# zjkang/Relation-DETR

Hardware: AMD Instinct MI355X
Metric: images/sec @ 800×1333, 300 queries, R50 4-level; achieved HBM GB/s (higher is better)
Workload: dtype bf16; 1 GPU; relation_detr_resnet50_800_1333 transformer stack from feature pyramids: 6 encoder layers (MSDA self-attn, S=22323, 4 levels) + two-stage top-k + 6 decoder layers (relation-biased self-attn + MSDA cross-attn + box refinement) + top-300 detections; backbone/neck excluded; batch_per_gpu=4, global_batch=4, queries=900, levels=4, launch=hipGraph replay, streams=2, gemm_tuning=False, parallelism=image-parallel x1

## Files before the change

include/relation_detr_amd.h:

```cpp
#ifndef RELATION_DETR_AMD_H
#define RELATION_DETR_AMD_H

#include <stdint.h>

#ifdef __cplusplus
extern "C" {
#endif

#define RDETR_ABI_VERSION 3

typedef enum rdetr_status {
    RDETR_OK = 0,
    RDETR_ERR_INVALID_ARG = -1,
    RDETR_ERR_UNSUPPORTED = -2,
    RDETR_ERR_LAUNCH = -3
} rdetr_status;

int rdetr_abi_version(void);
const char *rdetr_status_string(int status);

int rdetr_msda_forward_f32(const float *value, const int64_t *spatial_shapes, const int64_t *level_start_index,
                           const float *sampling_loc, const float *attn_weight, int B, int S, int H, int D,
                           int L, int Nq, int P, float *out, void *stream);

// ... 58 lines not shown
                                   int D, uint16_t *dst, void *stream);

int rdetr_linear_k256_hm_bf16(const uint16_t *x, long long ldx, const uint16_t *w, const uint16_t *bias, const uint8_t *row_mask,
                              int B, int S, uint16_t *out_hm, void *stream);

int rdetr_msda_fast_path(int H, int D, int L, int P);

int rdetr_msda_backward_f32(const float *value, const int64_t *spatial_shapes, const int64_t *level_start_index,
                            const float *sampling_loc, const float *attn_weight, const float *grad_out, int B,
                            int S, int H, int D, int L, int Nq, int P, float *grad_value,
                            float *grad_sampling_loc, float *grad_attn_weight, void *stream);

long long rdetr_msda_backward_det_workspace_bytes(int B, int S, int H, int D, int L, int Nq, int P);
int rdetr_msda_backward_det_f32(const float *value, const int64_t *spatial_shapes, const int64_t *level_start_index,
                                const float *sampling_loc, const float *attn_weight, const float *grad_out, int B, int S, int H, int D,
                                int L, int Nq, int P, void *workspace, long long workspace_bytes, float *grad_value,
                                float *grad_sampling_loc, float *grad_attn_weight, void *stream);

int rdetr_msda_backward_fused_f32(const float *value, const int64_t *spatial_shapes, const int64_t *level_start_index,
                                  const float *sampling_offsets, const float *attn_logits, const float *reference_points, int ref_dim,
                                  const float *grad_out, int B, int S, int H, int D, int L, int Nq, int P, void *workspace,
                                  long long workspace_bytes, float *grad_value, float *grad_offsets, float *grad_logits,
                                  float *grad_ref_partial, void *stream);
int rdetr_msda_backward_fused_bf16(const uint16_t *value, const int64_t *spatial_shapes, const int64_t *level_start_index,
                                   const uint16_t *sampling_offsets, const uint16_t *attn_logits, const float *reference_points,
                                   int ref_dim, const uint16_t *grad_out, int B, int S, int H, int D, int L, int Nq, int P,
                                   void *workspace, long long workspace_bytes, float *grad_value, uint16_t *grad_offsets,
                                   uint16_t *grad_logits, float *grad_ref_partial, void *stream);

int rdetr_relation_bias_f32(const float *src, const float *tgt, const float *proj_weight, const float *proj_bias,
                            int B, int N1, int N2, int Hh, int F, float scale, float temperature, float eps,
                            float *out, void *stream);

int rdetr_relation_bias_ws_f32(const float *src, const float *tgt, const float *proj_weight, const float *proj_bias,
                               int B, int N1, int N2, int Hh, int F, float scale, float temperature, float eps,
                               float *workspace, float *out, void *stream);

long long rdetr_relation_bias_backward_workspace_bytes(int B, int N1, int N2);
int rdetr_relation_bias_backward_f32(const float *src, const float *tgt, const float *grad_out, const uint8_t *active, int B, int N1,
                                     int N2, int Hh, int F, float scale, float temperature, float eps, float *workspace,
                                     float *grad_weight, float *grad_bias, void *stream);

int rdetr_bias_softmax_f32(float *scores, const float *bias, const uint8_t *mask, int BH, int N1, int N2,
                           void *stream);

int rdetr_relation_attention_bf16(const uint16_t *q, const uint16_t *k, const uint16_t *v, int ldq, int ldk, int ldv,
                                  const float *bias, const uint8_t *bool_mask, int B, int H, int D, int N, int M,
                                  float scale, uint16_t *out, int ldo, void *stream);

int rdetr_relation_attention_train_bf16(const uint16_t *q, const uint16_t *k, const uint16_t *v, int ldq, int ldk, int ldv,
                                        const float *bias, const uint8_t *bool_mask, int B, int H, int D, int N, int M,
                                        float scale, uint16_t *out, int ldo, float *lse, void *stream);

long long rdetr_relation_attention_backward_workspace_bytes(int B, int H, int N);
int rdetr_relation_attention_backward_bf16(const uint16_t *q, const uint16_t *k, const uint16_t *v, int ldq, int ldk, int ldv,
                                           const uint16_t *out, int ldo, const float *lse, const uint16_t *dout, int lddo,
                                           const float *bias, const uint8_t *bool_mask, int B, int H, int D, int N, int M,
                                           float scale, void *workspace, long long workspace_bytes, uint16_t *dq, int lddq,
                                           uint16_t *dk, int lddk, uint16_t *dv, int lddv, float *dbias, void *stream);

int rdetr_relation_attention_boxes_bf16(const uint16_t *q, const uint16_t *k, const uint16_t *v, int ldq, int ldk, int ldv,
                                        const float *src_boxes, const float *tgt_boxes, const float *proj_weight,
                                        const float *proj_bias, const uint8_t *bool_mask, int B, int H, int D,
                                        int N, int M, int F, float rel_scale, float temperature, float eps, float attn_scale,
                                        uint16_t *out, int ldo, void *stream);

int rdetr_relation_attention_boxes_train_bf16(const uint16_t *q, const uint16_t *k, const uint16_t *v, int ldq, int ldk, int ldv,
                                              const float *src_boxes, const float *tgt_boxes, const float *proj_weight,
                                              const float *proj_bias, const uint8_t *bool_mask, int B, int H, int D,
                                              int N, int M, int F, float rel_scale, float temperature, float eps, float attn_scale,
                                              uint16_t *out, int ldo, float *lse, void *stream);

long long rdetr_relation_attention_boxes_backward_workspace_bytes(int B, int H, int N, int M);
int rdetr_relation_attention_boxes_backward_bf16(const uint16_t *q, const uint16_t *k, const uint16_t *v, int ldq, int ldk, int ldv,
                                                 const uint16_t *out, int ldo, const float *lse, const uint16_t *dout, int lddo,
                                                 const float *src_boxes, const float *tgt_boxes, const float *proj_weight,
                                                 const float *proj_bias, const uint8_t *bool_mask, int B, int H, int D, int N, int M,
                                                 int F, float rel_scale, float temperature, float eps, float attn_scale,
                                                 void *workspace, long long workspace_bytes, uint16_t *dq, int lddq, uint16_t *dk,
                                                 int lddk, uint16_t *dv, int lddv, float *grad_weight, float *grad_bias,
                                                 void *stream);

int rdetr_add_layernorm_f32(const float *x, const float *residual, const float *gamma, const float *beta,
                            long long rows, int C, float eps, float *out, void *stream);
int rdetr_add_layernorm_bf16(const uint16_t *x, const uint16_t *residual, const uint16_t *gamma, const uint16_t *beta,
                             long long rows, int C, float eps, uint16_t *out, void *stream);
int rdetr_add_layernorm_strided_f32(const float *x, const float *residual, const float *gamma, const float *beta,
                                    long long rows, int C, long long ldx, long long ldr, long long ldo, float eps,
                                    float *out, void *stream);
int rdetr_add_layernorm_strided_bf16(const uint16_t *x, const uint16_t *residual, const uint16_t *gamma,
                                     const uint16_t *beta, long long rows, int C, long long ldx, long long ldr,
                                     long long ldo, float eps, uint16_t *out, void *stream);

int rdetr_add_layernorm_pos_f32(const float *x, const float *residual, const float *gamma, const float *beta,
                                const float *pos, long long rows, int C, long long ldx, long long ldr, long long ldo,
                                long long ldp, long long ldo2, float eps, float *out, float *out2, void *stream);
int rdetr_add_layernorm_pos_bf16(const uint16_t *x, const uint16_t *residual, const uint16_t *gamma,
                                 const uint16_t *beta, const uint16_t *pos, long long rows, int C, long long ldx,
                                 long long ldr, long long ldo, long long ldp, long long ldo2, float eps, uint16_t *out,
                                 uint16_t *out2, void *stream);

int rdetr_box_refine_f32(const void *delta, int delta_is_bf16, const float *ref, long long n, float eps, float *out,
                         void *stream);
int rdetr_sine_pos_embed(const float *pos, long long rows, int n, int F, float temperature, float scale, void *out,
                         int out_is_bf16, void *stream);

int rdetr_zero_masked_rows(void *x, const unsigned char *mask, long long rows, int row_bytes, long long ld_bytes,
                           void *stream);
int rdetr_row_max(const void *x, int is_bf16, long long rows, int C, long long ldx, void *out, void *stream);

long long rdetr_topk_workspace_bytes(int rows, int n, int k);
int rdetr_topk(const void *x, int is_bf16, int rows, int n, int k, void *workspace, float *values, long long *indices, void *stream);

int rdetr_box_head_k256_bf16(const uint16_t *xa, long long lda, const uint16_t *xb, long long ldb, const uint16_t *pw1,
                             const uint16_t *b1, const uint16_t *pw2, const uint16_t *b2, const uint16_t *w3, const uint16_t *b3,
                             const float *reference, int reference_is_logit, float eps, long long M, float *out_a, float *out_b,
                             void *stream);

int rdetr_query_pos_k256_bf16(const uint16_t *emb, long long lde, const uint16_t *query, long long ldq, const uint16_t *pw1a,
                              const uint16_t *pw1b, const uint16_t *b1, const uint16_t *pw2, const uint16_t *b2, const uint16_t *pv1,
                              const uint16_t *c1, const uint16_t *pv2, const uint16_t *c2, long long M, uint16_t *out_pos,
                              uint16_t *out_qpp, void *stream);

int rdetr_encoder_proj_k256_bf16(const uint16_t *x, long long ldx, const uint16_t *xq, long long ldq, const uint16_t *pwv,
                                 const uint16_t *bv, const uint16_t *pwq, const uint16_t *bq, const uint8_t *row_mask, int B, int S,
                                 int q_cols, uint16_t *out_hm, uint16_t *out_q, void *stream);

int rdetr_detections_from_topk(const float *score, const long long *index, const float *boxes, const long long *image_sizes, int B,
                               int N, int C, int K, float *out, void *stream);

int rdetr_scaled_pos(const void *a, const void *scale, const void *query, long long n, int is_bf16, void *pos, void *qp, void *stream);

int rdetr_decoder_reference(const float *reference, const float *valid_ratios, int B, int N, int L, int F, float temperature,
                            float scale, float *ref_in, void *emb, int emb_is_bf16, void *stream);

int rdetr_pyramid_points(const unsigned char *const *level_masks, const int *level_hw, int L, int B, const unsigned char *pad_mask,
                         int keep_is_bf16, float *valid_ratios, float *reference, float *logit, void *keep, void *stream);
int rdetr_nchw_to_tokens(const void *src, const void *add_vec, int is_bf16, int B, int C, int P,
                         long long out_image_stride, long long ld_out, void *out, void *stream);
int rdetr_nchw_levels_to_tokens(const void *const *level_src, const void *const *level_vec, const int *level_pixels, int L,
                                int is_bf16, int B, int C, long long out_image_stride, long long ld_out, void *out, void *stream);

int rdetr_linear_k256_bf16(const uint16_t *x, long long ldx, const uint16_t *w, const uint16_t *bias, long long M, int N,
                           int relu, uint16_t *out, long long ldo, void *stream);

int rdetr_linear_pack_k256_bf16(const uint16_t *w, uint16_t *packed, void *stream);
int rdetr_linear_ln_k256_bf16(const uint16_t *x, long long ldx, const uint16_t *packed, const uint16_t *bias,
                              const uint16_t *residual, long long ldr, const uint16_t *gamma, const uint16_t *beta, float eps,
                              long long M, uint16_t *out, long long ldo, void *stream);

int rdetr_ffn_k256_pack_bf16(const uint16_t *w1, const uint16_t *w2, int F, uint16_t *packed, void *stream);
int rdetr_ffn_k256_bf16(const uint16_t *x, long long ldx, const uint16_t *packed, const uint16_t *b1, const uint16_t *b2,
                        long long M, int F, uint16_t *out, long long ldo, void *stream);
int rdetr_ffn_ln_k256_bf16(const uint16_t *x, long long ldx, const uint16_t *packed, const uint16_t *b1, const uint16_t *b2,
                           const uint16_t *gamma, const uint16_t *beta, float eps, const uint16_t *pos, long long ldp,
                           long long M, int F, uint16_t *out, long long ldo, uint16_t *out2, long long ldo2, void *stream);
int rdetr_ffn_k256_train_bf16(const uint16_t *x, long long ldx, const uint16_t *packed, const uint16_t *b1, const uint16_t *b2,
                              long long M, int F, uint16_t *out, long long ldo, uint16_t *hid, long long ldh, void *stream);
int rdetr_ffn_k256_backward_bf16(const uint16_t *dy, long long lddy, const uint16_t *packed_t, const uint16_t *hid, long long ldh,
                                 long long M, int F, uint16_t *dh, long long ldd, uint16_t *dx, long long lddx, void *stream);

#ifdef __cplusplus
}
#endif
#endif
```

relation_detr_amd/_lib.py:

```python
from __future__ import annotations

import ctypes
import os

_HERE = os.path.dirname(os.path.abspath(__file__))
LIB_PATH = os.environ.get("RDETR_LIB_PATH") or os.path.join(_HERE, "librelation_detr_amd.so")

_c_int, _c_float, _vp, _c_ll = ctypes.c_int, ctypes.c_float, ctypes.c_void_p, ctypes.c_longlong

SIGNATURES = {
    "rdetr_abi_version": [],
    "rdetr_status_string": [_c_int],
    "rdetr_msda_fast_path": [_c_int] * 4,
    "rdetr_msda_levels_window_ok": [_vp, _vp, _c_int, _c_ll],
    "rdetr_msda_forward_f32": [_vp] * 5 + [_c_int] * 7 + [_vp, _vp],
    "rdetr_msda_forward_bf16": [_vp] * 5 + [_c_int] * 7 + [_vp, _vp],
    "rdetr_msda_forward_fused_f32": [_vp] * 6 + [_c_int] * 8 + [_vp, _vp],
    "rdetr_msda_forward_fused_bf16": [_vp] * 6 + [_c_int] * 8 + [_vp, _vp],
    "rdetr_msda_forward_fused_ex_f32": [_vp] * 4 + [_c_int, _vp, _c_int, _vp, _c_int, _vp] + [_c_int] * 7 + [_vp, _vp],
    "rdetr_msda_forward_fused_ex_bf16": [_vp] * 4 + [_c_int, _vp, _c_int, _vp, _c_int, _vp] + [_c_int] * 7 + [_vp, _vp],
    "rdetr_msda_forward_opt_bf16": [_vp, _c_int] + [_vp] * 4 + [_c_int] * 8 + [_vp, _vp],
    "rdetr_msda_forward_sweep_bf16": [_vp, _c_int] + [_vp] * 4 + [_c_int] * 7 + [_vp, _vp],
    "rdetr_msda_forward_resident_bf16": [_vp] * 5 + [_c_int] * 7 + [_vp, _vp],
    "rdetr_msda_forward_fused_resident_bf16": [_vp, _vp, _vp, _vp, _c_int, _vp, _c_int, _vp, _c_int] + [_c_int] * 7 + [_vp, _vp],
    "rdetr_msda_forward_fused_opt_bf16": [_vp, _c_int, _vp, _vp, _vp, _c_int, _vp, _c_int, _vp, _c_int, _vp] + [_c_int] * 8 + [_vp, _vp],
    "rdetr_msda_forward_fused_strided_bf16": [_vp, _c_ll, _vp, _vp, _vp, _c_int, _vp, _c_int, _vp, _c_int, _vp] + [_c_int] * 7 + [_vp, _vp],
    "rdetr_value_to_head_major_bf16": [_vp, _c_ll, _vp] + [_c_int] * 4 + [_vp, _vp],
    "rdetr_msda_backward_f32": [_vp] * 6 + [_c_int] * 7 + [_vp] * 4,
    "rdetr_msda_backward_det_workspace_bytes": [_c_int] * 7,
    "rdetr_msda_backward_det_f32": [_vp] * 6 + [_c_int] * 7 + [_vp, _c_ll] + [_vp] * 4,
    "rdetr_msda_backward_fused_f32": [_vp] * 6 + [_c_int, _vp] + [_c_int] * 7 + [_vp, _c_ll] + [_vp] * 5,
    "rdetr_msda_backward_fused_bf16": [_vp] * 6 + [_c_int, _vp] + [_c_int] * 7 + [_vp, _c_ll] + [_vp] * 5,
    "rdetr_relation_bias_f32": [_vp] * 4 + [_c_int] * 5 + [_c_float] * 3 + [_vp, _vp],
    "rdetr_relation_bias_ws_f32": [_vp] * 4 + [_c_int] * 5 + [_c_float] * 3 + [_vp, _vp, _vp],
    "rdetr_relation_bias_backward_workspace_bytes": [_c_int] * 3,
    "rdetr_relation_bias_backward_f32": [_vp] * 4 + [_c_int] * 5 + [_c_float] * 3 + [_vp] * 4,
    "rdetr_bias_softmax_f32": [_vp] * 3 + [_c_int] * 3 + [_vp],
    "rdetr_relation_attention_bf16": [_vp] * 3 + [_c_int] * 3 + [_vp, _vp] + [_c_int] * 5 + [_c_float, _vp, _c_int, _vp],
    "rdetr_relation_attention_train_bf16": [_vp] * 3 + [_c_int] * 3 + [_vp, _vp] + [_c_int] * 5 + [_c_float, _vp, _c_int, _vp, _vp],
    "rdetr_relation_attention_backward_workspace_bytes": [_c_int] * 3,
    "rdetr_relation_attention_backward_bf16": [_vp] * 3 + [_c_int] * 3 + [_vp, _c_int, _vp, _vp, _c_int, _vp, _vp] + [_c_int] * 5
                                              + [_c_float, _vp, _c_ll] + [_vp, _c_int] * 3 + [_vp, _vp],
    "rdetr_relation_attention_boxes_bf16": [_vp] * 3 + [_c_int] * 3 + [_vp] * 5 + [_c_int] * 6 + [_c_float] * 4 + [_vp, _c_int, _vp],
    "rdetr_relation_attention_boxes_train_bf16": [_vp] * 3 + [_c_int] * 3 + [_vp] * 5 + [_c_int] * 6 + [_c_float] * 4
                                                 + [_vp, _c_int, _vp, _vp],
    "rdetr_relation_attention_boxes_backward_workspace_bytes": [_c_int] * 4,
    "rdetr_relation_attention_boxes_backward_bf16": [_vp] * 3 + [_c_int] * 3 + [_vp, _c_int, _vp, _vp, _c_int] + [_vp] * 5 + [_c_int] * 6
                                                    + [_c_float] * 4 + [_vp, _c_ll] + [_vp, _c_int] * 3 + [_vp, _vp, _vp],
    "rdetr_box_refine_f32": [_vp, _c_int, _vp, _c_ll, _c_float, _vp, _vp],
    "rdetr_sine_pos_embed": [_vp, _c_ll, _c_int, _c_int, _c_float, _c_float, _vp, _c_int, _vp],
    "rdetr_zero_masked_rows": [_vp, _vp, _c_ll, _c_int, _c_ll, _vp],
    "rdetr_row_max": [_vp, _c_int, _c_ll, _c_int, _c_ll, _vp, _vp],
    "rdetr_topk_workspace_bytes": [_c_int, _c_int, _c_int],
    "rdetr_topk": [_vp, _c_int, _c_int, _c_int, _c_int, _vp, _vp, _vp, _vp],
    "rdetr_box_head_k256_bf16": [_vp, _c_ll, _vp, _c_ll, _vp, _vp, _vp, _vp, _vp, _vp, _vp, _c_int, _c_float, _c_ll, _vp, _vp, _vp],
    "rdetr_query_pos_k256_bf16": [_vp, _c_ll, _vp, _c_ll] + [_vp] * 9 + [_c_ll, _vp, _vp, _vp],
    "rdetr_encoder_proj_k256_bf16": [_vp, _c_ll, _vp, _c_ll] + [_vp] * 5 + [_c_int, _c_int, _c_int, _vp, _vp, _vp],
    "rdetr_detections_from_topk": [_vp, _vp, _vp, _vp, _c_int, _c_int, _c_int, _c_int, _vp, _vp],
    "rdetr_scaled_pos": [_vp, _vp, _vp, _c_ll, _c_int, _vp, _vp, _vp],
    "rdetr_decoder_reference": [_vp, _vp, _c_int, _c_int, _c_int, _c_int, _c_float, _c_float, _vp, _vp, _c_int, _vp],
    "rdetr_pyramid_points": [_vp, _vp, _c_int, _c_int, _vp, _c_int, _vp, _vp, _vp, _vp, _vp],
    "rdetr_linear_k256_bf16": [_vp, _c_ll, _vp, _vp, _c_ll, _c_int, _c_int, _vp, _c_ll, _vp],
    "rdetr_linear_k256_hm_bf16": [_vp, _c_ll, _vp, _vp, _vp, _c_int, _c_int, _vp, _vp],
    "rdetr_linear_pack_k256_bf16": [_vp, _vp, _vp],
    "rdetr_linear_ln_k256_bf16": [_vp, _c_ll, _vp, _vp, _vp, _c_ll, _vp, _vp, _c_float, _c_ll, _vp, _c_ll, _vp],
    "rdetr_ffn_k256_pack_bf16": [_vp, _vp, _c_int, _vp, _vp],
    "rdetr_ffn_k256_bf16": [_vp, _c_ll, _vp, _vp, _vp, _c_ll, _c_int, _vp, _c_ll, _vp],
    "rdetr_ffn_ln_k256_bf16": [_vp, _c_ll, _vp, _vp, _vp, _vp, _vp, _c_float, _vp, _c_ll, _c_ll, _c_int, _vp, _c_ll, _vp, _c_ll, _vp],
    "rdetr_ffn_k256_train_bf16": [_vp, _c_ll, _vp, _vp, _vp, _c_ll, _c_int, _vp, _c_ll, _vp, _c_ll, _vp],
    "rdetr_ffn_k256_backward_bf16": [_vp, _c_ll, _vp, _vp, _c_ll, _c_ll, _c_int, _vp, _c_ll, _vp, _c_ll, _vp],
    "rdetr_nchw_to_tokens": [_vp, _vp, _c_int, _c_int, _c_int, _c_int, _c_ll, _c_ll, _vp, _vp],
    "rdetr_nchw_levels_to_tokens": [_vp, _vp, _vp, _c_int, _c_int, _c_int, _c_int, _c_ll, _c_ll, _vp, _vp],
    "rdetr_add_layernorm_f32": [_vp] * 4 + [_c_ll, _c_int, _c_float, _vp, _vp],
    "rdetr_add_layernorm_bf16": [_vp] * 4 + [_c_ll, _c_int, _c_float, _vp, _vp],
    "rdetr_add_layernorm_strided_f32": [_vp] * 4 + [_c_ll, _c_int, _c_ll, _c_ll, _c_ll, _c_float, _vp, _vp],
    "rdetr_add_layernorm_strided_bf16": [_vp] * 4 + [_c_ll, _c_int, _c_ll, _c_ll, _c_ll, _c_float, _vp, _vp],
    "rdetr_add_layernorm_pos_f32": [_vp] * 5 + [_c_ll, _c_int] + [_c_ll] * 5 + [_c_float, _vp, _vp, _vp],
    "rdetr_add_layernorm_pos_bf16": [_vp] * 5 + [_c_ll, _c_int] + [_c_ll] * 5 + [_c_float, _vp, _vp, _vp],
}

ERR_INVALID_ARG, ERR_UNSUPPORTED, ERR_LAUNCH = -1, -2, -3

_lib = None


class RdetrError(RuntimeError):
    pass


def load() -> ctypes.CDLL:
    global _lib
    if _lib is not None:
        return _lib
    if not os.path.exists(LIB_PATH):
        raise RdetrError(
            f"{LIB_PATH} not found: the HIP kernels are not built. Run `make -C relation_detr_amd/csrc` "
            "(needs hipcc, --offload-arch=gfx950). There is no CPU or PyTorch fallback for this path.")
    lib = ctypes.CDLL(LIB_PATH)
    for name, argtypes in SIGNATURES.items():
        fn = getattr(lib, name)
        fn.argtypes = argtypes
        fn.restype = ctypes.c_char_p if name == "rdetr_status_string" else (_c_ll if name.endswith("_workspace_bytes") else _c_int)
    if lib.rdetr_abi_version() != 3:
        raise RdetrError(f"ABI version mismatch: library {lib.rdetr_abi_version()}, binding 3")
    _lib = lib
    return lib


def check(status: int, what: str) -> None:
    if status != 0:
        msg = load().rdetr_status_string(status).decode()
        raise RdetrError(f"{what} failed: {msg} (status {status})")
```

relation_detr_amd/ops.py:

```python
from __future__ import annotations

import collections
import weakref
from typing import Optional, Tuple

import torch

from . import _lib


_KEEP: "collections.deque" = collections.deque(maxlen=64)


def _cptr(t: torch.Tensor) -> int:
    if t.is_contiguous():
        return t.data_ptr()
    c = t.contiguous()
    _KEEP.append(c)
    return c.data_ptr()


def _stream_ptr(t: torch.Tensor) -> int:
    return torch.cuda.current_stream(t.device).cuda_stream

# ... 1042 lines not shown
    L, B = len(level_masks), level_masks[0].shape[0]
    masks = [m.contiguous() for m in level_masks]
    if any(m.dtype != torch.bool or m.dim() != 3 or m.shape[0] != B for m in masks) or keep_dtype not in (torch.float32, torch.bfloat16):
        raise _lib.RdetrError("pyramid_points: bool masks [B, h, w] per level, keep in float32 or bfloat16")
    S = sum(m.shape[1] * m.shape[2] for m in masks)
    dev = masks[0].device
    pad = None
    if pad_mask is not None:
        if tuple(pad_mask.shape) != (B, S) or pad_mask.dtype != torch.bool:
            raise _lib.RdetrError("pyramid_points: pad_mask must be bool [B, S]")
        pad = pad_mask.contiguous()
    ptrs = (ctypes.c_void_p * L)(*[m.data_ptr() for m in masks])
    hw = (ctypes.c_int * (2 * L))(*[v for m in masks for v in (m.shape[1], m.shape[2])])
    ratios = torch.empty(B, L, 2, dtype=torch.float32, device=dev)
    reference = torch.empty(B, S, L, 2, dtype=torch.float32, device=dev)
    logit = torch.empty(B, S, 4, dtype=torch.float32, device=dev)
    keep = torch.empty(B, S, dtype=keep_dtype, device=dev)
    st = _lib.load().rdetr_pyramid_points(ptrs, hw, L, B, None if pad is None else pad.data_ptr(), int(keep_dtype == torch.bfloat16),
                                          ratios.data_ptr(), reference.data_ptr(), logit.data_ptr(), keep.data_ptr(), _stream_ptr(ratios))
    _lib.check(st, "rdetr_pyramid_points")
    return ratios, reference, logit, keep


def tokens_from_levels(levels, add_vecs=None, out: Optional[torch.Tensor] = None) -> torch.Tensor:
    x0 = levels[0]
    _require_device(*levels)
    B, C = x0.shape[:2]
    S = sum(x.shape[2] * x.shape[3] for x in levels)
    if out is None:
        out = torch.empty(B, S, C, dtype=x0.dtype, device=x0.device)
    if tuple(out.shape) != (B, S, C) or out.dtype != x0.dtype or out.stride(-1) != 1 or (B > 1 and out.stride(0) < S * out.stride(1)):
        raise _lib.RdetrError("tokens_from_levels: out must be [B, S, C] in the levels' dtype with contiguous channels")
    lib, es, row = _lib.load(), out.element_size(), 0
    xs, vecs = [], []
    for l, x in enumerate(levels):
        if x.shape[:2] != (B, C) or x.dtype != x0.dtype:
            raise _lib.RdetrError("tokens_from_levels: levels must agree in batch, channels and dtype")
        xs.append(x.contiguous())
        vec = None
        if add_vecs is not None:
            vec = add_vecs[l].to(x0.dtype).contiguous()
            if vec.numel() != C:
                raise _lib.RdetrError("tokens_from_levels: add_vecs[l] needs C entries")
        vecs.append(vec)
    L = len(xs)
    if L <= 8:
        import ctypes
        src = (ctypes.c_void_p * L)(*[x.data_ptr() for x in xs])
        vp = (ctypes.c_void_p * L)(*[None if v is None else v.data_ptr() for v in vecs])
        pix = (ctypes.c_int * L)(*[x.shape[2] * x.shape[3] for x in xs])
        st = lib.rdetr_nchw_levels_to_tokens(src, vp, pix, L, int(x0.dtype == torch.bfloat16), B, C, out.stride(0), out.stride(1),
                                             out.data_ptr(), _stream_ptr(x0))
        _lib.check(st, "rdetr_nchw_levels_to_tokens")
        return out
    for x, vec in zip(xs, vecs):
        P = x.shape[2] * x.shape[3]
        st = lib.rdetr_nchw_to_tokens(x.data_ptr(), vec.data_ptr() if vec is not None else None, int(x0.dtype == torch.bfloat16),
                                      B, C, P, out.stride(0), out.stride(1), out.data_ptr() + row * out.stride(1) * es,
                                      _stream_ptr(x0))
        _lib.check(st, "rdetr_nchw_to_tokens")
        row += P
    return out


def linear_k256_supported(x: torch.Tensor, weight: torch.Tensor) -> bool:
    if not (x.is_cuda and x.dtype == torch.bfloat16 and weight.dtype == torch.bfloat16 and x.shape[-1] == 256
            and weight.dim() == 2 and weight.shape[1] == 256 and weight.shape[0] % 32 == 0 and weight.is_contiguous()):
        return False
    try:
        _, _, ld = _rows_view(x, "linear_k256")
    except _lib.RdetrError:
        return False
    return ld % 8 == 0 and x.data_ptr() % 16 == 0 and weight.data_ptr() % 16 == 0


def linear_k256(x: torch.Tensor, weight: torch.Tensor, bias: Optional[torch.Tensor] = None, relu: bool = False,
                out: Optional[torch.Tensor] = None) -> torch.Tensor:
    _require_device(x, weight, bias, out)
    if not linear_k256_supported(x, weight):
        raise _lib.RdetrError("linear_k256: needs bf16, K = 256, N % 32 == 0, evenly strided 16-byte aligned rows")
    rows, _, ldx = _rows_view(x, "linear_k256")
    N = weight.shape[0]
    if bias is not None and (bias.dtype != torch.bfloat16 or bias.numel() != N):
        raise _lib.RdetrError("linear_k256: bias must be bf16 [N]")
    if out is None:
        out = torch.empty(*x.shape[:-1], N, dtype=x.dtype, device=x.device)
    elif tuple(out.shape) != (*x.shape[:-1], N) or out.dtype != x.dtype:
        raise _lib.RdetrError("linear_k256: out must be [..., N] bf16")
    orows, _, ldo = _rows_view(out, "linear_k256")
    if orows != rows or ldo % 8 or out.data_ptr() % 16:
        raise _lib.RdetrError("linear_k256: out rows must be 16-byte aligned")
    st = _lib.load().rdetr_linear_k256_bf16(x.data_ptr(), ldx, weight.data_ptr(), None if bias is None else _cptr(bias),
                                            rows, N, int(relu), out.data_ptr(), ldo, _stream_ptr(x))
    _lib.check(st, "rdetr_linear_k256_bf16")
    return out


def value_proj_head_major(x: torch.Tensor, weight: torch.Tensor, bias: Optional[torch.Tensor],
                          key_padding_mask: Optional[torch.Tensor] = None) -> torch.Tensor:
    _require_device(x, weight, bias, key_padding_mask)
    if x.dim() != 3 or not linear_k256_supported(x, weight) or tuple(weight.shape) != (256, 256):
        raise _lib.RdetrError("value_proj_head_major: needs bf16 x [B, S, 256] with evenly strided 16-byte aligned rows and a [256, 256] weight")
    B, S, _ = x.shape
    _, _, ldx = _rows_view(x, "value_proj_head_major")
    if bias is not None and (bias.dtype != torch.bfloat16 or bias.numel() != 256):
        raise _lib.RdetrError("value_proj_head_major: bias must be bf16 [256]")
    mask_ptr = None
    if key_padding_mask is not None:
        if tuple(key_padding_mask.shape) != (B, S):
            raise _lib.RdetrError("key_padding_mask must be [B, S]")
        mask_u8 = key_padding_mask.contiguous().view(torch.uint8) if key_padding_mask.dtype == torch.bool \
            else key_padding_mask.to(torch.uint8).contiguous()
        mask_ptr = mask_u8.data_ptr()
    out = torch.empty(B, 8, S, 32, dtype=torch.bfloat16, device=x.device)
    st = _lib.load().rdetr_linear_k256_hm_bf16(x.data_ptr(), ldx, weight.data_ptr(), None if bias is None else _cptr(bias),
                                               mask_ptr, B, S, out.data_ptr(), _stream_ptr(x))
    _lib.check(st, "rdetr_linear_k256_hm_bf16")
    return out


def ffn_k256_supported(x: torch.Tensor, w1: torch.Tensor, w2: torch.Tensor) -> bool:
    F = w1.shape[0] if w1.dim() == 2 else 0
    return (linear_k256_supported(x, w1) and w2.dtype == torch.bfloat16 and tuple(w2.shape) == (256, F) and F % 64 == 0
            and F <= 4096 and w2.is_contiguous() and w2.data_ptr() % 16 == 0)


class _PackedWeightCache:

    def __init__(self, prune_every: int = 64):
        self._entries: dict = {}
        self._prune_every = prune_every
        self._misses = 0

    def get(self, tensors, build):
        key = tuple(id(t) for t in tensors)
        ver = tuple((t._version, tuple(t.shape), t.data_ptr(), t.device) for t in tensors)
        hit = self._entries.get(key)
        if hit is not None:
            refs, hver, packed = hit
            if hver == ver and all(r() is t for r, t in zip(refs, tensors)):
                return packed
        self._misses += 1
        if self._misses % self._prune_every == 0:
            self._entries = {k: v for k, v in self._entries.items() if all(r() is not None for r in v[0])}
        packed = build()
        self._entries[key] = (tuple(weakref.ref(t) for t in tensors), ver, packed)
        return packed

    def __len__(self):
        return len(self._entries)


_FFN_PACKED = _PackedWeightCache()


def ffn_k256_packed_weights(w1: torch.Tensor, w2: torch.Tensor) -> torch.Tensor:
    def build():
        F = w1.shape[0]
        packed = torch.empty(2 * 256 * F, dtype=torch.bfloat16, device=w1.device)
        st = _lib.load().rdetr_ffn_k256_pack_bf16(w1.data_ptr(), w2.data_ptr(), F, packed.data_ptr(), _stream_ptr(w1))
        _lib.check(st, "rdetr_ffn_k256_pack_bf16")
        if not torch.cuda.is_current_stream_capturing():
            torch.cuda.current_stream(w1.device).synchronize()
        return packed
    return _FFN_PACKED.get((w1, w2), build)


def ffn_k256(x: torch.Tensor, w1: torch.Tensor, b1: torch.Tensor, w2: torch.Tensor, b2: torch.Tensor,
             out: Optional[torch.Tensor] = None) -> torch.Tensor:
    _require_device(x, w1, b1, w2, b2, out)
    if not ffn_k256_supported(x, w1, w2):
        raise _lib.RdetrError("ffn_k256: needs bf16, embed_dim 256, d_ffn % 64 == 0 (<= 4096), evenly strided 16-byte aligned rows")
    F = w1.shape[0]
    if b1.dtype != torch.bfloat16 or b2.dtype != torch.bfloat16 or b1.numel() != F or b2.numel() != 256:
        raise _lib.RdetrError("ffn_k256: biases must be bf16 [F] and [256]")
    rows, _, ldx = _rows_view(x, "ffn_k256")
    if out is None:
        out = torch.empty(*x.shape[:-1], 256, dtype=x.dtype, device=x.device)
    elif tuple(out.shape) != tuple(x.shape) or out.dtype != x.dtype:
        raise _lib.RdetrError("ffn_k256: out must have x's shape and dtype")
    orows, _, ldo = _rows_view(out, "ffn_k256")
    if orows != rows or ldo % 8 or out.data_ptr() % 16:
        raise _lib.RdetrError("ffn_k256: out rows must be 16-byte aligned")
    packed = ffn_k256_packed_weights(w1, w2)
    st = _lib.load().rdetr_ffn_k256_bf16(x.data_ptr(), ldx, packed.data_ptr(), _cptr(b1),
                                         _cptr(b2), rows, F, out.data_ptr(), ldo, _stream_ptr(x))
    _lib.check(st, "rdetr_ffn_k256_bf16")
    return out


def ffn_ln_k256(x: torch.Tensor, w1: torch.Tensor, b1: torch.Tensor, w2: torch.Tensor, b2: torch.Tensor, gamma: torch.Tensor,
                beta: torch.Tensor, eps: float = 1e-5, out: Optional[torch.Tensor] = None, pos: Optional[torch.Tensor] = None):
    _require_device(x, w1, b1, w2, b2, gamma, beta, out, pos)
    if not ffn_k256_supported(x, w1, w2):
        raise _lib.RdetrError("ffn_ln_k256: needs bf16, embed_dim 256, d_ffn % 64 == 0 (<= 4096), evenly strided 16-byte aligned rows")
    F = w1.shape[0]
    for t, n in ((b1, F), (b2, 256), (gamma, 256), (beta, 256)):
        if t.dtype != torch.bfloat16 or t.numel() != n:
            raise _lib.RdetrError("ffn_ln_k256: biases / LayerNorm parameters must be bf16 of the matching size")
    rows, _, ldx = _rows_view(x, "ffn_ln_k256")
    if out is None:
        out = torch.empty(*x.shape[:-1], 256, dtype=x.dtype, device=x.device)
    elif tuple(out.shape) != tuple(x.shape) or out.dtype != x.dtype:
        raise _lib.RdetrError("ffn_ln_k256: out must have x's shape and dtype")
    orows, _, ldo = _rows_view(out, "ffn_ln_k256")
    if orows != rows or ldo % 8 or out.data_ptr() % 16:
        raise _lib.RdetrError("ffn_ln_k256: out rows must be 16-byte aligned")
    out2, ldp = None, 0
    if pos is not None:
        if tuple(pos.shape) != tuple(x.shape) or pos.dtype != x.dtype:
            raise _lib.RdetrError("ffn_ln_k256: pos must have x's shape and dtype")
        prows, _, ldp = _rows_view(pos, "ffn_ln_k256")
        if ldp % 8 or pos.data_ptr() % 16:
            raise _lib.RdetrError("ffn_ln_k256: pos rows must be 16-byte aligned")
        out2 = torch.empty(*x.shape[:-1], 256, dtype=x.dtype, device=x.device)
    packed = ffn_k256_packed_weights(w1, w2)
    st = _lib.load().rdetr_ffn_ln_k256_bf16(x.data_ptr(), ldx, packed.data_ptr(), _cptr(b1), _cptr(b2),
                                            _cptr(gamma), _cptr(beta), float(eps),
                                            None if pos is None else pos.data_ptr(), ldp, rows, F, out.data_ptr(), ldo,
                                            None if out2 is None else out2.data_ptr(), 256, _stream_ptr(x))
    _lib.check(st, "rdetr_ffn_ln_k256_bf16")
    return out if pos is None else (out, out2)


_LINEAR_PACKED = _PackedWeightCache()
_REL_PROJ_F32 = _PackedWeightCache()


def linear_ln_k256_supported(x: torch.Tensor, weight: torch.Tensor, residual: torch.Tensor) -> bool:
    if not (linear_k256_supported(x, weight) and tuple(weight.shape) == (256, 256) and residual.dtype == torch.bfloat16
            and residual.is_cuda and tuple(residual.shape) == tuple(x.shape)):
        return False
    try:
        _, _, ldr = _rows_view(residual, "linear_ln_k256")
    except _lib.RdetrError:
        return False
    return ldr % 8 == 0 and residual.data_ptr() % 16 == 0


def linear_ln_k256(x: torch.Tensor, weight: torch.Tensor, bias: Optional[torch.Tensor], residual: torch.Tensor,
                   gamma: torch.Tensor, beta: torch.Tensor, eps: float = 1e-5, out: Optional[torch.Tensor] = None) -> torch.Tensor:
    _require_device(x, weight, bias, residual, gamma, beta, out)
    if not linear_ln_k256_supported(x, weight, residual):
        raise _lib.RdetrError("linear_ln_k256: needs bf16 [..., 256] inputs with evenly strided 16-byte aligned rows and a [256, 256] weight")
    for t in (bias, gamma, beta):
        if t is not None and (t.dtype != torch.bfloat16 or t.numel() != 256):
            raise _lib.RdetrError("linear_ln_k256: bias / gamma / beta must be bf16 [256]")
    rows, _, ldx = _rows_view(x, "linear_ln_k256")
    _, _, ldr = _rows_view(residual, "linear_ln_k256")
    if out is None:
        out = torch.empty(x.shape, dtype=x.dtype, device=x.device)
    elif tuple(out.shape) != tuple(x.shape) or out.dtype != x.dtype:
        raise _lib.RdetrError("linear_ln_k256: out must have x's shape and dtype")
    orows, _, ldo = _rows_view(out, "linear_ln_k256")
    if orows != rows or ldo % 8 or out.data_ptr() % 16:
        raise _lib.RdetrError("linear_ln_k256: out rows must be 16-byte aligned")
    lib = _lib.load()
    def build():
        packed = torch.empty(256 * 256, dtype=torch.bfloat16, device=weight.device)
        _lib.check(lib.rdetr_linear_pack_k256_bf16(weight.data_ptr(), packed.data_ptr(), _stream_ptr(weight)), "rdetr_linear_pack_k256_bf16")
        if not torch.cuda.is_current_stream_capturing():
            torch.cuda.current_stream(weight.device).synchronize()
        return packed
    packed_w = _LINEAR_PACKED.get((weight,), build)
    st = lib.rdetr_linear_ln_k256_bf16(x.data_ptr(), ldx, packed_w.data_ptr(), None if bias is None else _cptr(bias),
                                       residual.data_ptr(), ldr, _cptr(gamma), _cptr(beta),
                                       float(eps), rows, out.data_ptr(), ldo, _stream_ptr(x))
    _lib.check(st, "rdetr_linear_ln_k256_bf16")
    return out
```

relation_detr_amd/transformer.py:

```python
from __future__ import annotations

import math
from typing import List, Sequence

import torch
from torch import Tensor, nn
from torch.nn import functional as F

from . import ffn_train, ops
from . import options as _options
from .ms_deform_attn import MultiScaleDeformableAttention
from .relation import PositionRelationEmbedding
from .self_attn import RelationSelfAttention


def inverse_sigmoid(x: Tensor, eps: float = 1e-3) -> Tensor:
    x = x.clamp(min=0, max=1)
    return torch.log(x.clamp(min=eps) / (1 - x).clamp(min=eps))


def refine_boxes(delta: Tensor, reference: Tensor) -> Tensor:
    if delta.is_cuda and reference.dtype == torch.float32 and not (torch.is_grad_enabled() and delta.requires_grad):
        from . import ops
        return ops.box_refine(delta, reference)
    return (delta.float() + inverse_sigmoid(reference)).sigmoid()


def sine_pos_embed(pos: Tensor, num_pos_feats: int = 128, temperature: float = 10000.0,
                   scale: float = 2 * math.pi) -> Tensor:
    k = torch.arange(num_pos_feats // 2, dtype=torch.float32, device=pos.device)
    dim_t = temperature ** (k * 2 / num_pos_feats)
    ang = pos.unsqueeze(-1) * scale / dim_t
    emb = torch.stack((ang.sin(), ang.cos()), dim=-1).flatten(-2)
    return torch.cat((emb[..., 1:2, :], emb[..., 0:1, :], emb[..., 2:, :]), dim=-2).flatten(-2)


def add_norm(norm: nn.LayerNorm, x: Tensor, residual: Tensor = None, out: Tensor = None) -> Tensor:
    needs_grad = torch.is_grad_enabled() and (x.requires_grad or norm.weight.requires_grad or
                                              (residual is not None and residual.requires_grad))
    if x.is_cuda and not needs_grad and x.dtype in (torch.float32, torch.bfloat16):
        from . import ops
        return ops.add_layer_norm(x, residual, norm.weight, norm.bias, norm.eps, out=out)
    y = norm(x if residual is None else x + residual)
    if out is not None:
        out.copy_(y)
        return out
    return y


_K256_MIN_ROWS = 16384


def linear_relu(linear: nn.Linear, x: Tensor, opts: "_options.Options" = None) -> Tensor:
    if x.is_cuda and linear.bias is not None and not (torch.is_grad_enabled() and (x.requires_grad or linear.weight.requires_grad)):
        rows = x.numel() // x.shape[-1]
        if (rows >= _K256_MIN_ROWS and linear.out_features >= 1024 and (opts or _options.get()).linear_k256
                and not torch.is_grad_enabled() and ops.linear_k256_supported(x, linear.weight)):
            return ops.linear_k256(x, linear.weight, linear.bias, relu=True)
        y = torch._addmm_activation(linear.bias, x.reshape(-1, x.shape[-1]), linear.weight.t(), use_gelu=False)
        return y.view(*x.shape[:-1], linear.out_features)
    return F.relu(linear(x))


def _fused_ffn_applies(linear1: nn.Linear, linear2: nn.Linear, x: Tensor, opts: "_options.Options" = None) -> bool:
    return (x.is_cuda and not torch.is_grad_enabled() and x.numel() // x.shape[-1] >= _K256_MIN_ROWS
            and linear1.bias is not None and linear2.bias is not None and (opts or _options.get()).ffn_fused
            and ops.ffn_k256_supported(x, linear1.weight, linear2.weight))


def _fused_ffn_train_applies(linear1: nn.Linear, linear2: nn.Linear, x: Tensor, opts: "_options.Options" = None) -> bool:
    if not ((opts or _options.get()).ffn_train_fused and x.is_cuda and torch.is_grad_enabled()
            and linear1.bias is not None and linear2.bias is not None and x.numel() // x.shape[-1] >= _K256_MIN_ROWS):
        return False
    params = (linear1.weight, linear1.bias, linear2.weight, linear2.bias)
    return ((x.requires_grad or any(p.requires_grad for p in params))
            and ffn_train.ffn_train_supported(x, linear1.weight, linear1.bias, linear2.weight, linear2.bias))


def feed_forward(linear1: nn.Linear, linear2: nn.Linear, x: Tensor, opts: "_options.Options" = None) -> Tensor:
    if _fused_ffn_applies(linear1, linear2, x, opts):
        return ops.ffn_k256(x, linear1.weight, linear1.bias, linear2.weight, linear2.bias)
    if _fused_ffn_train_applies(linear1, linear2, x, opts):
        return ffn_train.FeedForwardFunction.apply(x, linear1.weight, linear1.bias, linear2.weight, linear2.bias)
    return linear2(linear_relu(linear1, x, opts))


class MLP(nn.Module):

    def __init__(self, input_dim: int, hidden_dim: int, output_dim: int, num_layers: int):
        super().__init__()
        dims = [input_dim] + [hidden_dim] * (num_layers - 1) + [output_dim]
        self.num_layers = num_layers
        self.options = _options.get()
        self.layers = nn.ModuleList(nn.Linear(a, b) for a, b in zip(dims[:-1], dims[1:]))
        for layer in self.layers:
            nn.init.xavier_uniform_(layer.weight)
            nn.init.zeros_(layer.bias)

    def forward(self, x: Tensor) -> Tensor:
        for i, layer in enumerate(self.layers):
            x = linear_relu(layer, x, self.options) if i + 1 < self.num_layers else layer(x)
        return x


class RelationTransformerEncoderLayer(nn.Module):
    def __init__(self, embed_dim=256, d_ffn=1024, n_heads=8, n_levels=4, n_points=4, msda_cls=MultiScaleDeformableAttention):
        super().__init__()
        self.embed_dim = embed_dim
        self.options = _options.get()
        self.self_attn = msda_cls(embed_dim, n_levels, n_heads, n_points)
        self.norm1 = nn.LayerNorm(embed_dim)
        self.linear1 = nn.Linear(embed_dim, d_ffn)
        self.linear2 = nn.Linear(d_ffn, embed_dim)
        self.norm2 = nn.LayerNorm(embed_dim)
        nn.init.xavier_uniform_(self.linear1.weight)
        nn.init.xavier_uniform_(self.linear2.weight)

    def forward(self, query, query_pos, reference_points, spatial_shapes, level_start_index, key_padding_mask=None, out=None,
                query_plus_pos=None, next_pos=None):
        if query_plus_pos is None:
            query_plus_pos = query if query_pos is None else query + query_pos
        if type(self.self_attn).forward is MultiScaleDeformableAttention.forward:
            query = self.self_attn(query=query_plus_pos, reference_points=reference_points, value=query,
                                   spatial_shapes=spatial_shapes, level_start_index=level_start_index,
                                   key_padding_mask=key_padding_mask, post_norm=(query, self.norm1))
        else:
            attn = self.self_attn(query=query_plus_pos, reference_points=reference_points,
                                  value=query, spatial_shapes=spatial_shapes, level_start_index=level_start_index,
                                  key_padding_mask=key_padding_mask)
            query = add_norm(self.norm1, query, attn)
        if self.options.ffn_ln and _fused_ffn_applies(self.linear1, self.linear2, query, self.options):
            return ops.ffn_ln_k256(query, self.linear1.weight, self.linear1.bias, self.linear2.weight, self.linear2.bias,
                                   self.norm2.weight, self.norm2.bias, self.norm2.eps, out=out, pos=next_pos)
        ffn = feed_forward(self.linear1, self.linear2, query, self.options)
        if next_pos is not None:
            return ops.add_layer_norm(query, ffn, self.norm2.weight, self.norm2.bias, self.norm2.eps, out=out, pos=next_pos)
        return add_norm(self.norm2, query, ffn, out=out)


class RelationTransformerEncoder(nn.Module):

    def __init__(self, layers: Sequence[RelationTransformerEncoderLayer]):
        super().__init__()
        self.layers = nn.ModuleList(layers)
        self.num_layers = len(self.layers)
        self.embed_dim = self.layers[0].embed_dim
        self.options = _options.get()
        d = self.embed_dim
        self.memory_fusion = nn.Sequential(nn.Linear((self.num_layers + 1) * d, d), nn.ReLU(inplace=True), nn.Linear(d, d),
                                           nn.LayerNorm(d))

    def forward(self, query, spatial_shapes, level_start_index, reference_points, query_pos=None, query_key_padding_mask=None,
                fusion_buffer=None):
        fuse = self.memory_fusion
        if query.is_cuda and not torch.is_grad_enabled():
            d = self.embed_dim
            if fusion_buffer is not None:
                stacked = fusion_buffer
            else:
                stacked = torch.empty(*query.shape[:-1], (self.num_layers + 1) * d, dtype=query.dtype, device=query.device)
                stacked[..., :d].copy_(query)
            query = stacked[..., :d]
            fuse_pos = (query_pos is not None and query.dtype in (torch.float32, torch.bfloat16)
                        and self.options.ln_pos)
            qpp = None
            for i, layer in enumerate(self.layers):
                last = i + 1 == self.num_layers
                res = layer(query, query_pos, reference_points, spatial_shapes, level_start_index, query_key_padding_mask,
                            out=stacked[..., (i + 1) * d:(i + 2) * d], query_plus_pos=qpp,
                            next_pos=query_pos if fuse_pos and not last else None)
                query, qpp = res if isinstance(res, tuple) else (res, None)
            return add_norm(fuse[3], fuse[2](linear_relu(fuse[0], stacked, self.options)))
        outs = [query]
        for layer in self.layers:
            query = layer(query, query_pos, reference_points, spatial_shapes, level_start_index, query_key_padding_mask)
            outs.append(query)
        return add_norm(fuse[3], fuse[2](linear_relu(fuse[0], torch.cat(outs, -1), self.options)))


class RelationTransformerDecoderLayer(nn.Module):
    def __init__(self, embed_dim=256, d_ffn=1024, n_heads=8, n_levels=4, n_points=4,
                 msda_cls=MultiScaleDeformableAttention, self_attn_cls=RelationSelfAttention):
        super().__init__()
        self.embed_dim, self.num_heads = embed_dim, n_heads
        self.options = _options.get()
        self.cross_attn = msda_cls(embed_dim, n_levels, n_heads, n_points)
        self.norm1 = nn.LayerNorm(embed_dim)
        self.self_attn = self_attn_cls(embed_dim, n_heads, dropout=0.0, batch_first=True)
        self.norm2 = nn.LayerNorm(embed_dim)
        self.linear1 = nn.Linear(embed_dim, d_ffn)
        self.linear2 = nn.Linear(d_ffn, embed_dim)
        self.norm3 = nn.LayerNorm(embed_dim)
        nn.init.xavier_uniform_(self.linear1.weight)
        nn.init.xavier_uniform_(self.linear2.weight)

    def forward(self, query, query_pos, reference_points, value, spatial_shapes, level_start_index, self_attn_mask=None,
                key_padding_mask=None, query_plus_pos=None, projected_value=None):
        qp = query + query_pos if query_plus_pos is None else query_plus_pos
        attn = self.self_attn(query=qp, key=qp, value=query, attn_mask=self_attn_mask, need_weights=False)[0]
        if (query.is_cuda and not torch.is_grad_enabled() and query.dtype in (torch.float32, torch.bfloat16)
                and query_pos.dtype == query.dtype and query_pos.shape == query.shape and self.options.decoder_ln_pos):
            query, cross_q = ops.add_layer_norm(attn, query, self.norm2.weight, self.norm2.bias, self.norm2.eps, pos=query_pos)
        else:
            query = add_norm(self.norm2, query, attn)
            cross_q = query + query_pos
        cross = self.cross_attn(query=cross_q, reference_points=reference_points, value=value,
                                spatial_shapes=spatial_shapes, level_start_index=level_start_index,
                                key_padding_mask=key_padding_mask,
                                **({} if projected_value is None else {"projected_value": projected_value}))
        query = add_norm(self.norm1, query, cross)
        return add_norm(self.norm3, query, feed_forward(self.linear1, self.linear2, query, self.options))


class RelationTransformerDecoder(nn.Module):

    def __init__(self, layers: Sequence[RelationTransformerDecoderLayer], num_classes: int,
                 relation_cls=PositionRelationEmbedding):
        super().__init__()
# ... 303 lines not shown
```

Before: 1083 images/s.

## Add split-F fused FFN kernel with reduction for short row counts

Adds a fused FFN kernel for small row counts (up to 2048 rows, such as decoder queries). It splits the hidden dimension F across grid slices, writes fp32 partial sums to a workspace, and finishes with a separate reduction kernel that adds the slices and converts to bf16. The goal is to fill the GPU when M is too small for the row-tiled fused kernel, which the decoder FFN previously did not use at all. In exchange it adds a second launch, an fp32 workspace round trip, and a per-call torch.empty allocation.

```diff
diff --git a/include/relation_detr_amd.h b/include/relation_detr_amd.h
--- a/include/relation_detr_amd.h
+++ b/include/relation_detr_amd.h
@@ -234,6 +234,9 @@
 int rdetr_ffn_k256_pack_bf16(const uint16_t *w1, const uint16_t *w2, int F, uint16_t *packed, void *stream);
 int rdetr_ffn_k256_bf16(const uint16_t *x, long long ldx, const uint16_t *packed, const uint16_t *b1, const uint16_t *b2,
                         long long M, int F, uint16_t *out, long long ldo, void *stream);
+long long rdetr_ffn_k256_short_workspace_bytes(long long M, int F);
+int rdetr_ffn_k256_short_bf16(const uint16_t *x, long long ldx, const uint16_t *packed, const uint16_t *b1, const uint16_t *b2,
+                              long long M, int F, uint16_t *out, long long ldo, void *workspace, void *stream);
 int rdetr_ffn_ln_k256_bf16(const uint16_t *x, long long ldx, const uint16_t *packed, const uint16_t *b1, const uint16_t *b2,
                            const uint16_t *gamma, const uint16_t *beta, float eps, const uint16_t *pos, long long ldp,
                            long long M, int F, uint16_t *out, long long ldo, uint16_t *out2, long long ldo2, void *stream);
diff --git a/relation_detr_amd/_lib.py b/relation_detr_amd/_lib.py
--- a/relation_detr_amd/_lib.py
+++ b/relation_detr_amd/_lib.py
@@ -66,6 +66,8 @@
     "rdetr_linear_ln_k256_bf16": [_vp, _c_ll, _vp, _vp, _vp, _c_ll, _vp, _vp, _c_float, _c_ll, _vp, _c_ll, _vp],
     "rdetr_ffn_k256_pack_bf16": [_vp, _vp, _c_int, _vp, _vp],
     "rdetr_ffn_k256_bf16": [_vp, _c_ll, _vp, _vp, _vp, _c_ll, _c_int, _vp, _c_ll, _vp],
+    "rdetr_ffn_k256_short_workspace_bytes": [_c_ll, _c_int],
+    "rdetr_ffn_k256_short_bf16": [_vp, _c_ll, _vp, _vp, _vp, _c_ll, _c_int, _vp, _c_ll, _vp, _vp],
     "rdetr_ffn_ln_k256_bf16": [_vp, _c_ll, _vp, _vp, _vp, _vp, _vp, _c_float, _vp, _c_ll, _c_ll, _c_int, _vp, _c_ll, _vp, _c_ll, _vp],
     "rdetr_ffn_k256_train_bf16": [_vp, _c_ll, _vp, _vp, _vp, _c_ll, _c_int, _vp, _c_ll, _vp, _c_ll, _vp],
     "rdetr_ffn_k256_backward_bf16": [_vp, _c_ll, _vp, _vp, _c_ll, _c_ll, _c_int, _vp, _c_ll, _vp, _c_ll, _vp],
diff --git a/relation_detr_amd/csrc/ffn_short.hip b/relation_detr_amd/csrc/ffn_short.hip
--- /dev/null
+++ b/relation_detr_amd/csrc/ffn_short.hip
@@ -0,0 +1,184 @@
+#include "common.h"
+
+namespace rdetr {
+
+typedef __bf16 ffs_bf16x8 __attribute__((ext_vector_type(8)));
+
+constexpr int kFfsWaves = 8, kFfsThreads = kFfsWaves * 64;
+constexpr int kFfsRound = 256;
+
+template <int NB, int NQ>
+__global__ __launch_bounds__(kFfsThreads) void ffn_k256_short_partial_kernel(const uint16_t *__restrict__ x, long long ldx,
+                                                                             const uint16_t *__restrict__ packed,
+                                                                             const uint16_t *__restrict__ b1,
+                                                                             const uint16_t *__restrict__ b2, long long M, int F,
+                                                                             float *__restrict__ ws)
+{
+    constexpr int kImg = NB * 8 * 64;
+    __shared__ __attribute__((aligned(16))) u32x4 img[NQ * kImg];
+    const int tid = threadIdx.x, lane = tid & 63, wave = __builtin_amdgcn_readfirstlane(tid >> 6);
+    const int col = lane & 15, g = lane >> 4;
+    const long long row0 = (long long)blockIdx.x * (16 * NB) + col;
+    const int nchunk = F >> 6;
+    const u32x4 *pk = reinterpret_cast<const u32x4 *>(packed) + lane;
+
+    struct Frags { u32x4 f[16]; };
+    auto fetch1 = [&](int q, Frags &w) {
+        int c = (blockIdx.y * NQ + q) * 4 + (wave >> 1);
+        c = c < nchunk ? c : nchunk - 1;
+        const u32x4 *p = pk + (size_t)c * 64 * 64;
+#pragma unroll
+        for (int i = 0; i < 16; ++i) w.f[i] = p[((2 * (wave & 1) + (i & 1)) * 8 + (i >> 1)) * 64];
+        __builtin_amdgcn_sched_barrier(0);
+    };
+    auto fetch2 = [&](int q, Frags &w) {
+#pragma unroll
+        for (int i = 0; i < 16; ++i) {
+            int c = (blockIdx.y * NQ + q) * 4 + (i >> 2);
+            c = c < nchunk ? c : nchunk - 1;
+            w.f[i] = pk[((size_t)c * 64 + 32 + 2 * (2 * wave + (i & 1)) + ((i >> 1) & 1)) * 64];
+        }
+        __builtin_amdgcn_sched_barrier(0);
+    };
+    auto mm = [&](const u32x4 &a, const u32x4 &bq, const f32x4 &c) {
+        return __builtin_amdgcn_mfma_f32_16x16x32_bf16(__builtin_bit_cast(ffs_bf16x8, a), __builtin_bit_cast(ffs_bf16x8, bq), c, 0, 0, 0);
+    };
+
+    Frags w1, w2;
+    fetch1(0, w1);
+    u32x4 xr[NB][8];
+#pragma unroll
+    for (int cb = 0; cb < NB; ++cb) {
+        const long long r = row0 + 16 * cb < M ? row0 + 16 * cb : M - 1;
+        const uint16_t *p = x + r * ldx + 8 * g;
+#pragma unroll
+        for (int s = 0; s < 8; ++s) xr[cb][s] = *reinterpret_cast<const u32x4 *>(p + 32 * s);
+    }
+    fetch2(0, w2);
+    __builtin_amdgcn_sched_barrier(0);
+
+    f32x4 out_acc[2][NB];
+#pragma unroll
+    for (int e = 0; e < 2; ++e) {
+        f32x4 b4 = {0.f, 0.f, 0.f, 0.f};
+        if (blockIdx.y == 0) {
+            const uint16_t *bp = b2 + 32 * wave + 8 * g + 4 * e;
+            b4 = f32x4{bf16_bits_to_f32(bp[0]), bf16_bits_to_f32(bp[1]), bf16_bits_to_f32(bp[2]), bf16_bits_to_f32(bp[3])};
+        }
+#pragma unroll
+        for (int cb = 0; cb < NB; ++cb) out_acc[e][cb] = b4;
+    }
+
+#pragma unroll
+    for (int q = 0; q < NQ; ++q) {
+        const int h0 = (blockIdx.y * NQ + q) * kFfsRound;
+        if (q > 0) {
+            if (h0 >= F) break;
+            fetch1(q, w1);
+            fetch2(q, w2);
+        }
+        u32x4 *image = img + q * kImg;
+        const bool mine = h0 + 32 * wave < F;
+        if (mine) {
+            const uint16_t *bp = b1 + h0 + 32 * wave + 8 * g;
+            const f32x4 blo = {bf16_bits_to_f32(bp[0]), bf16_bits_to_f32(bp[1]), bf16_bits_to_f32(bp[2]), bf16_bits_to_f32(bp[3])};
+            const f32x4 bhi = {bf16_bits_to_f32(bp[4]), bf16_bits_to_f32(bp[5]), bf16_bits_to_f32(bp[6]), bf16_bits_to_f32(bp[7])};
+            f32x4 acc[2][NB];
+#pragma unroll
+            for (int e = 0; e < 2; ++e)
+#pragma unroll
+                for (int cb = 0; cb < NB; ++cb) acc[e][cb] = f32x4{0.f, 0.f, 0.f, 0.f};
+#pragma unroll
+            for (int i = 0; i < 16; ++i)
+#pragma unroll
+                for (int cb = 0; cb < NB; ++cb) acc[i & 1][cb] = mm(w1.f[i], xr[cb][i >> 1], acc[i & 1][cb]);
+#pragma unroll
+            for (int cb = 0; cb < NB; ++cb) {
+                const f32x4 lo = acc[0][cb] + blo, hi = acc[1][cb] + bhi;
+                image[(cb * 8 + wave) * 64 + lane] = u32x4{relu_bf16x2(pack_bf16x2(lo.x, lo.y)), relu_bf16x2(pack_bf16x2(lo.z, lo.w)),
+                                                           relu_bf16x2(pack_bf16x2(hi.x, hi.y)), relu_bf16x2(pack_bf16x2(hi.z, hi.w))};
+            }
+        } else {
+#pragma unroll
+            for (int cb = 0; cb < NB; ++cb) image[(cb * 8 + wave) * 64 + lane] = u32x4{0u, 0u, 0u, 0u};
+        }
+        __syncthreads();
+#pragma unroll
+        for (int s = 0; s < 8; ++s) {
+            if (h0 + 32 * s >= F) break;
+#pragma unroll
+            for (int cb = 0; cb < NB; ++cb) {
+                const u32x4 y = image[(cb * 8 + s) * 64 + lane];
+                out_acc[0][cb] = mm(w2.f[2 * s], y, out_acc[0][cb]);
+                out_acc[1][cb] = mm(w2.f[2 * s + 1], y, out_acc[1][cb]);
+            }
+        }
+    }
+    float *wp = ws + (size_t)blockIdx.y * (size_t)M * 256 + 32 * wave + 8 * g;
+#pragma unroll
+    for (int cb = 0; cb < NB; ++cb) {
+        const long long r = row0 + 16 * cb;
+        if (r < M) {
+            *reinterpret_cast<f32x4 *>(wp + r * 256) = out_acc[0][cb];
+            *reinterpret_cast<f32x4 *>(wp + r * 256 + 4) = out_acc[1][cb];
+        }
+    }
+}
+
+__global__ __launch_bounds__(256) void ffn_k256_short_reduce_kernel(const float *__restrict__ ws, int S, long long M,
+                                                                    uint16_t *__restrict__ out, long long ldo)
+{
+    const long long idx = (long long)blockIdx.x * 256 + threadIdx.x;
+    const long long row = idx >> 5;
+    const int c = (int)(idx & 31) * 8;
+    if (row >= M) return;
+    const float *p = ws + row * 256 + c;
+    f32x4 lo = *reinterpret_cast<const f32x4 *>(p), hi = *reinterpret_cast<const f32x4 *>(p + 4);
+    for (int s = 1; s < S; ++s) {
+        p += (size_t)M * 256;
+        lo += *reinterpret_cast<const f32x4 *>(p);
+        hi += *reinterpret_cast<const f32x4 *>(p + 4);
+    }
+    const u32x4 o = {pack_bf16x2(lo.x, lo.y), pack_bf16x2(lo.z, lo.w), pack_bf16x2(hi.x, hi.y), pack_bf16x2(hi.z, hi.w)};
+    *reinterpret_cast<u32x4 *>(out + row * ldo + c) = o;
+}
+
+constexpr int kFfsNB = 2;
+constexpr long long kFfsOneRoundMaxRows = 1024;
+
+static int ffs_rounds(long long M) { return M <= kFfsOneRoundMaxRows ? 1 : 2; }
+static int ffs_slices(long long M, int F) { return (F + kFfsRound * ffs_rounds(M) - 1) / (kFfsRound * ffs_rounds(M)); }
+
+}
+
+using namespace rdetr;
+
+extern "C" long long rdetr_ffn_k256_short_workspace_bytes(long long M, int F)
+{
+    if (M <= 0 || F <= 0) return 0;
+    return (long long)ffs_slices(M, F) * M * 256 * 4;
+}
+
+extern "C" int rdetr_ffn_k256_short_bf16(const uint16_t *x, long long ldx, const uint16_t *packed, const uint16_t *b1, const uint16_t *b2,
+                                         long long M, int F, uint16_t *out, long long ldo, void *workspace, void *stream)
+{
+    if (M < 0 || F <= 0 || ldx < 256 || ldo < 256) return RDETR_ERR_INVALID_ARG;
+    if ((F % 64) || F > 4096 || (ldx & 7) || (ldo & 7)) return RDETR_ERR_UNSUPPORTED;
+    if (M == 0) return RDETR_OK;
+    if (!x || !packed || !b1 || !b2 || !out || !workspace) return RDETR_ERR_INVALID_ARG;
+    if ((reinterpret_cast<uintptr_t>(x) | reinterpret_cast<uintptr_t>(packed) | reinterpret_cast<uintptr_t>(out) |
+         reinterpret_cast<uintptr_t>(workspace)) & 15)
+        return RDETR_ERR_UNSUPPORTED;
+    if (M > (1ll << 24)) return RDETR_ERR_UNSUPPORTED;
+    hipStream_t st = static_cast<hipStream_t>(stream);
+    float *ws = static_cast<float *>(workspace);
+    const int S = ffs_slices(M, F);
+    const dim3 grid((unsigned)((M + 16 * kFfsNB - 1) / (16 * kFfsNB)), (unsigned)S);
+    if (ffs_rounds(M) == 1)
+        hipLaunchKernelGGL((ffn_k256_short_partial_kernel<kFfsNB, 1>), grid, dim3(kFfsThreads), 0, st, x, ldx, packed, b1, b2, M, F, ws);
+    else
+        hipLaunchKernelGGL((ffn_k256_short_partial_kernel<kFfsNB, 2>), grid, dim3(kFfsThreads), 0, st, x, ldx, packed, b1, b2, M, F, ws);
+    if (launch_status() != RDETR_OK) return RDETR_ERR_LAUNCH;
+    hipLaunchKernelGGL(ffn_k256_short_reduce_kernel, dim3((unsigned)((M * 32 + 255) / 256)), dim3(256), 0, st, ws, S, M, out, ldo);
+    return launch_status();
+}
diff --git a/relation_detr_amd/ops.py b/relation_detr_amd/ops.py
--- a/relation_detr_amd/ops.py
+++ b/relation_detr_amd/ops.py
@@ -1218,6 +1218,7 @@
 
 
 _FFN_PACKED = _PackedWeightCache()
+_FFN_SHORT_MAX_ROWS = 2048
 
 
 def ffn_k256_packed_weights(w1: torch.Tensor, w2: torch.Tensor) -> torch.Tensor:
@@ -1249,8 +1250,15 @@
     if orows != rows or ldo % 8 or out.data_ptr() % 16:
         raise _lib.RdetrError("ffn_k256: out rows must be 16-byte aligned")
     packed = ffn_k256_packed_weights(w1, w2)
-    st = _lib.load().rdetr_ffn_k256_bf16(x.data_ptr(), ldx, packed.data_ptr(), _cptr(b1),
-                                         _cptr(b2), rows, F, out.data_ptr(), ldo, _stream_ptr(x))
+    lib = _lib.load()
+    if 0 < rows <= _FFN_SHORT_MAX_ROWS:
+        ws = torch.empty(lib.rdetr_ffn_k256_short_workspace_bytes(rows, F) // 4, dtype=torch.float32, device=x.device)
+        st = lib.rdetr_ffn_k256_short_bf16(x.data_ptr(), ldx, packed.data_ptr(), _cptr(b1), _cptr(b2), rows, F, out.data_ptr(), ldo,
+                                           ws.data_ptr(), _stream_ptr(x))
+        _lib.check(st, "rdetr_ffn_k256_short_bf16")
+        return out
+    st = lib.rdetr_ffn_k256_bf16(x.data_ptr(), ldx, packed.data_ptr(), _cptr(b1),
+                                 _cptr(b2), rows, F, out.data_ptr(), ldo, _stream_ptr(x))
     _lib.check(st, "rdetr_ffn_k256_bf16")
     return out
 
diff --git a/relation_detr_amd/transformer.py b/relation_detr_amd/transformer.py
--- a/relation_detr_amd/transformer.py
+++ b/relation_detr_amd/transformer.py
@@ -49,6 +49,7 @@
 
 
 _K256_MIN_ROWS = 16384
+_FFN_SHORT_MAX_ROWS = ops._FFN_SHORT_MAX_ROWS
 
 
 def linear_relu(linear: nn.Linear, x: Tensor, opts: "_options.Options" = None) -> Tensor:
@@ -63,7 +64,8 @@
 
 
 def _fused_ffn_applies(linear1: nn.Linear, linear2: nn.Linear, x: Tensor, opts: "_options.Options" = None) -> bool:
-    return (x.is_cuda and not torch.is_grad_enabled() and x.numel() // x.shape[-1] >= _K256_MIN_ROWS
+    rows = x.numel() // x.shape[-1]
+    return (x.is_cuda and not torch.is_grad_enabled() and (rows >= _K256_MIN_ROWS or 0 < rows <= _FFN_SHORT_MAX_ROWS)
             and linear1.bias is not None and linear2.bias is not None and (opts or _options.get()).ffn_fused
             and ops.ffn_k256_supported(x, linear1.weight, linear2.weight))
 
```

Result: slower. 1072 images/s (-1.1%).
